# Caxson/mere-fusion

Measured on AMD Instinct MI355X. Metric: lip-sync frames/sec @256x256, higher is better.
Workload: dtype bf16x3+f16q; 1 GPU; MuseTalk step 256x256: pe(audio) + UNet(t=0) + VAE decode to uint8 frames, batch=8 latents + Whisper chunks per GPU, inputs resident in HBM (BASELINE.json configs[2]); assumed MuseTalk-v1 / sd-vae-ft-mse architecture, seeded random-init weights; batch_per_gpu=8, parallelism=1 independent replicas, sessions sharded by GPU, no collective

## Files before the change

### mere-fusion_amd/csrc/mf_attn.hip

```cpp
#include "mf_nn.h"
#include <cmath>
#include <cstdlib>

typedef __attribute__((ext_vector_type(8))) __bf16 bf16x8;
typedef __attribute__((ext_vector_type(4))) short s16x4;
typedef __attribute__((ext_vector_type(8))) short s16x8;
typedef __attribute__((ext_vector_type(4))) float f32x4;
typedef __attribute__((ext_vector_type(4))) unsigned u32x4;
typedef __attribute__((ext_vector_type(2))) unsigned u32x2;

struct AttnArgs {
    const bf16_t *q_hi, *q_lo, *k_hi, *k_lo, *v_hi, *v_lo;
    bf16_t *o_hi, *o_lo;
    int64_t q_b, k_b, v_b, o_b;
    int q_row, k_row, v_row, o_row;
    int Tq, Tk, heads, qtiles, total;
    float scale_log2e;
};

namespace {

__device__ __forceinline__ uint32_t f2bf_rne(float f) {
    return (uint32_t)__builtin_bit_cast(unsigned short, (__bf16)f);
}
__device__ __forceinline__ float bf2f_(uint32_t h16) { return __uint_as_float(h16 << 16); }

__device__ __forceinline__ s16x4 lds_tr16(const bf16_t* p) {
    return __builtin_amdgcn_ds_read_tr16_b64_v4i16((s16x4 __attribute__((address_space(3)))*)(p));
}

template <int DH, int QB, int KT, bool X3>
__global__ __launch_bounds__(256) void k_attention(const AttnArgs a) {
    constexpr int NP = X3 ? 2 : 1;
    constexpr int NK32 = (DH + 31) / 32;
    constexpr int DHP = NK32 * 32 + 8;
    constexpr int MB = (DH + 15) / 16;
    constexpr int KB = KT / 16;
    constexpr int CPR = DH / 8;
    constexpr int CH = KT * CPR;
    constexpr int RND = (CH + 255) / 256;
    static_assert(DH % 8 == 0, "head dim");
    static_assert(KT % 32 == 0, "key tile");

    __shared__ __attribute__((aligned(16))) bf16_t Ks[NP][KT][DHP];
    __shared__ __attribute__((aligned(16))) bf16_t Vs[NP][KT][DHP];

    const int tid = threadIdx.x, lane = tid & 63, l16 = lane & 15, g = lane >> 4;
    const int wave = __builtin_amdgcn_readfirstlane(tid >> 6);

    const int bid = blockIdx.x, nt = a.total;
    const int qq = nt >> 3, rr = nt & 7, xcd = bid & 7;
    const int t = (xcd < rr ? xcd * (qq + 1) : rr * (qq + 1) + (xcd - rr) * qq) + (bid >> 3);
    const int grp = t / a.qtiles, qt = t - grp * a.qtiles;
    const int b = grp / a.heads, h = grp - b * a.heads;

    const bf16_t* qp[NP] = {a.q_hi + b * a.q_b + h * DH};
    const bf16_t* kp[NP] = {a.k_hi + b * a.k_b + h * DH};
    const bf16_t* vp[NP] = {a.v_hi + b * a.v_b + h * DH};
    if constexpr (X3) {
        qp[1] = a.q_lo + b * a.q_b + h * DH;
        kp[1] = a.k_lo + b * a.k_b + h * DH;
        vp[1] = a.v_lo + b * a.v_b + h * DH;
    }

    for (int i = tid; i < NP * KT * (DHP - DH); i += 256) {
        const int r = i / (DHP - DH), c = DH + i - r * (DHP - DH);
        (&Ks[0][0][0])[r * DHP + c] = 0;
        (&Vs[0][0][0])[r * DHP + c] = 0;
    }

    const int q0 = qt * (64 * QB) + wave * (16 * QB);
    bf16x8 qf[NP][QB][NK32];
#pragma unroll
    for (int qb = 0; qb < QB; ++qb) {
        int qrow = q0 + qb * 16 + l16;
        qrow = qrow < a.Tq ? qrow : a.Tq - 1;
#pragma unroll
        for (int p = 0; p < NP; ++p) {
            const bf16_t* src = qp[p] + (int64_t)qrow * a.q_row;
#pragma unroll
            for (int ks = 0; ks < NK32; ++ks) {
// ... 28 lines not shown
#pragma unroll
        for (int r = 0; r < RND; ++r) {
            const int c = tid + r * 256;
            if (CH % 256 == 0 || c < CH) {
                const int row = c / CPR, col = c - row * CPR;
#pragma unroll
                for (int p = 0; p < NP; ++p) {
                    *reinterpret_cast<u32x4*>(&Ks[p][row][col * 8]) = pre[p][r];
                    *reinterpret_cast<u32x4*>(&Vs[p][row][col * 8]) = pre[NP + p][r];
                }
            }
        }
    };

    f32x4 oacc[MB][QB];
#pragma unroll
    for (int mb = 0; mb < MB; ++mb)
#pragma unroll
        for (int qb = 0; qb < QB; ++qb) oacc[mb][qb] = f32x4{0.f, 0.f, 0.f, 0.f};
    float m_run[QB], l_run[QB];
#pragma unroll
    for (int qb = 0; qb < QB; ++qb) { m_run[qb] = -INFINITY; l_run[qb] = 0.f; }

    const int ntiles = (a.Tk + KT - 1) / KT;
    load_tile(0);
    for (int tile = 0; tile < ntiles; ++tile) {
        __syncthreads();
        store_tile();
        __syncthreads();
        if (tile + 1 < ntiles) load_tile(tile + 1);

        f32x4 s[KB][QB];
#pragma unroll
        for (int kb = 0; kb < KB; ++kb) {
#pragma unroll
            for (int qb = 0; qb < QB; ++qb) s[kb][qb] = f32x4{0.f, 0.f, 0.f, 0.f};
            const int krow = kb * 16 + l16;
#pragma unroll
            for (int ks = 0; ks < NK32; ++ks) {
                const bf16x8 khi = *reinterpret_cast<const bf16x8*>(&Ks[0][krow][ks * 32 + g * 8]);
                bf16x8 klo;
                if constexpr (X3) klo = *reinterpret_cast<const bf16x8*>(&Ks[NP - 1][krow][ks * 32 + g * 8]);
#pragma unroll
                for (int qb = 0; qb < QB; ++qb) {
                    if constexpr (X3) {
                        s[kb][qb] = __builtin_amdgcn_mfma_f32_16x16x32_bf16(klo, qf[0][qb][ks], s[kb][qb], 0, 0, 0);
                        s[kb][qb] = __builtin_amdgcn_mfma_f32_16x16x32_bf16(khi, qf[NP - 1][qb][ks], s[kb][qb], 0, 0, 0);
                    }
                    s[kb][qb] = __builtin_amdgcn_mfma_f32_16x16x32_bf16(khi, qf[0][qb][ks], s[kb][qb], 0, 0, 0);
                }
            }
        }

        const bool last = (tile + 1) * KT > a.Tk;
#pragma unroll
        for (int qb = 0; qb < QB; ++qb) {
            float mx = -INFINITY;
#pragma unroll
            for (int kb = 0; kb < KB; ++kb)
#pragma unroll
                for (int i = 0; i < 4; ++i) {
                    float v = s[kb][qb][i] * a.scale_log2e;
                    if (last && tile * KT + kb * 16 + g * 4 + i >= a.Tk) v = -INFINITY;
                    s[kb][qb][i] = v;
                    mx = fmaxf(mx, v);
                }
            mx = fmaxf(mx, __shfl_xor(mx, 16));
            mx = fmaxf(mx, __shfl_xor(mx, 32));
            const float m_new = fmaxf(m_run[qb], mx);
            const float alpha = __builtin_amdgcn_exp2f(m_run[qb] - m_new);
            m_run[qb] = m_new;
            float ps = 0.f;
#pragma unroll
            for (int kb = 0; kb < KB; ++kb)
#pragma unroll
                for (int i = 0; i < 4; ++i) {
                    const float p = __builtin_amdgcn_exp2f(s[kb][qb][i] - m_new);
                    s[kb][qb][i] = p;
                    ps += p;
                }
            l_run[qb] = l_run[qb] * alpha + ps;
#pragma unroll
            for (int mb = 0; mb < MB; ++mb)
#pragma unroll
                for (int i = 0; i < 4; ++i) oacc[mb][qb][i] *= alpha;
        }

#pragma unroll
        for (int pi = 0; pi < KB / 2; ++pi) {
            s16x8 phi[QB], plo[QB];
#pragma unroll
            for (int qb = 0; qb < QB; ++qb)
#pragma unroll
                for (int j = 0; j < 8; ++j) {
                    const float p = s[2 * pi + (j >> 2)][qb][j & 3];
                    const uint32_t hb = f2bf_rne(p);
                    phi[qb][j] = (short)hb;
                    if constexpr (X3) plo[qb][j] = (short)f2bf_rne(p - bf2f_(hb));
                }
            const int vrow = pi * 32 + g * 4 + (l16 >> 2), vcol = (l16 & 3) * 4;
#pragma unroll
            for (int mb = 0; mb < MB; ++mb) {
                const s16x4 a0 = lds_tr16(&Vs[0][vrow][mb * 16 + vcol]);
                const s16x4 a1 = lds_tr16(&Vs[0][vrow + 16][mb * 16 + vcol]);
                const s16x8 vhi = {a0[0], a0[1], a0[2], a0[3], a1[0], a1[1], a1[2], a1[3]};
                s16x8 vlo;
                if constexpr (X3) {
                    const s16x4 b0 = lds_tr16(&Vs[NP - 1][vrow][mb * 16 + vcol]);
                    const s16x4 b1 = lds_tr16(&Vs[NP - 1][vrow + 16][mb * 16 + vcol]);
                    vlo = s16x8{b0[0], b0[1], b0[2], b0[3], b1[0], b1[1], b1[2], b1[3]};
                }
#pragma unroll
                for (int qb = 0; qb < QB; ++qb) {
                    if constexpr (X3) {
                        oacc[mb][qb] = __builtin_amdgcn_mfma_f32_16x16x32_bf16(__builtin_bit_cast(bf16x8, vlo), __builtin_bit_cast(bf16x8, phi[qb]), oacc[mb][qb], 0, 0, 0);
                        oacc[mb][qb] = __builtin_amdgcn_mfma_f32_16x16x32_bf16(__builtin_bit_cast(bf16x8, vhi), __builtin_bit_cast(bf16x8, plo[qb]), oacc[mb][qb], 0, 0, 0);
                    }
                    oacc[mb][qb] = __builtin_amdgcn_mfma_f32_16x16x32_bf16(__builtin_bit_cast(bf16x8, vhi), __builtin_bit_cast(bf16x8, phi[qb]), oacc[mb][qb], 0, 0, 0);
                }
            }
        }
    }

    bf16_t* oh = a.o_hi + b * a.o_b + h * DH;
    bf16_t* ol = X3 ? a.o_lo + b * a.o_b + h * DH : nullptr;
#pragma unroll
    for (int qb = 0; qb < QB; ++qb) {
        float l = l_run[qb];
        l += __shfl_xor(l, 16);
        l += __shfl_xor(l, 32);
        const float inv = 1.f / l;
        const int qrow = q0 + qb * 16 + l16;
        if (qrow >= a.Tq) continue;
#pragma unroll
        for (int mb = 0; mb < MB; ++mb) {
            const int d = mb * 16 + g * 4;
            if (d >= DH) continue;
            float v[4];
            uint32_t hb[4];
#pragma unroll
            for (int i = 0; i < 4; ++i) { v[i] = oacc[mb][qb][i] * inv; hb[i] = f2bf_rne(v[i]); }
            const int64_t o = (int64_t)qrow * a.o_row + d;
            *reinterpret_cast<u32x2*>(oh + o) = u32x2{hb[0] | (hb[1] << 16), hb[2] | (hb[3] << 16)};
            if constexpr (X3) {
                uint32_t lb[4];
#pragma unroll
                for (int i = 0; i < 4; ++i) lb[i] = f2bf_rne(v[i] - bf2f_(hb[i]));
                *reinterpret_cast<u32x2*>(ol + o) = u32x2{lb[0] | (lb[1] << 16), lb[2] | (lb[3] << 16)};
            }
        }
    }
}

template <int DH, int QB, int KT>
int launch_prec(const AttnArgs& a, bool x3, hipStream_t s) {
    if (x3)
        hipLaunchKernelGGL((k_attention<DH, QB, KT, true>), dim3(a.total), dim3(256), 0, s, a);
    else
        hipLaunchKernelGGL((k_attention<DH, QB, KT, false>), dim3(a.total), dim3(256), 0, s, a);
    MF_HIP(hipGetLastError());
    return MF_OK;
}

template <int DH, int KT>
int launch_qb(AttnArgs& a, int groups, bool x3, hipStream_t s) {
    const bool wide = (int64_t)groups * ((a.Tq + 127) / 128) >= 512;
    if (DH <= 80 && wide) {
        a.qtiles = (a.Tq + 127) / 128;
        a.total = groups * a.qtiles;
        return launch_prec<DH, (DH <= 80 ? 2 : 1), KT>(a, x3, s);
    }
    a.qtiles = (a.Tq + 63) / 64;
    a.total = groups * a.qtiles;
    return launch_prec<DH, 1, KT>(a, x3, s);
}

}

bool mf_attention_supported(int dh) { return dh == 40 || dh == 64 || dh == 80 || dh == 160; }

int mf_attention(const ActView& q, const ActView& k, const ActView& v, const ActView& out, int heads, int batch, int precision,
                 hipStream_t s, int tq, int tk) {
    const int C = q.C, dh = C / heads;
    MF_REQUIRE(heads > 0 && C % heads == 0 && k.C == C && v.C == C && out.C == C, "attention: channel mismatch");
    MF_REQUIRE(mf_attention_supported(dh), "attention: no fused kernel for head dim %d", dh);
    for (const ActBuf* b : {q.buf, k.buf, v.buf, out.buf})
        MF_REQUIRE(b->halo == 0 || b->H == 1, "attention: needs contiguous token buffers");
    MF_REQUIRE(q.coff % 8 == 0 && k.coff % 8 == 0 && v.coff % 8 == 0 && out.coff % 8 == 0, "attention: views must start on 8-channel groups");
    const bool x3 = precision == MF_PREC_BF16X3;
    AttnArgs a{};
    const int64_t qo = mf_interior(*q.buf) + q.coff, ko = mf_interior(*k.buf) + k.coff, vo = mf_interior(*v.buf) + v.coff,
                  oo = mf_interior(*out.buf) + out.coff;
    a.q_hi = q.buf->hi + qo; a.k_hi = k.buf->hi + ko; a.v_hi = v.buf->hi + vo; a.o_hi = out.buf->hi + oo;
    if (x3) {
        a.q_lo = q.buf->lo + qo; a.k_lo = k.buf->lo + ko; a.v_lo = v.buf->lo + vo; a.o_lo = out.buf->lo + oo;
    }
    a.q_b = q.buf->per_batch(); a.k_b = k.buf->per_batch(); a.v_b = v.buf->per_batch(); a.o_b = out.buf->per_batch();
    a.q_row = q.buf->C; a.k_row = k.buf->C; a.v_row = v.buf->C; a.o_row = out.buf->C;
    a.Tq = q.buf->H * q.buf->W; a.Tk = k.buf->H * k.buf->W; a.heads = heads;
    MF_REQUIRE(a.Tq > 0 && a.Tk > 0 && v.buf->H * v.buf->W == a.Tk && out.buf->H * out.buf->W == a.Tq, "attention: token count mismatch");
    MF_REQUIRE(tq >= 0 && tq <= a.Tq && tk >= 0 && tk <= a.Tk, "attention: prefix (%d queries, %d keys) exceeds the sequences (%d, %d)", tq, tk, a.Tq, a.Tk);
    if (tq > 0) a.Tq = tq;
    if (tk > 0) a.Tk = tk;
    a.scale_log2e = (float)(1.4426950408889634 / std::sqrt((double)dh));
    const int groups = batch * heads;
    switch (dh) {
        case 40: return launch_qb<40, 64>(a, groups, x3, s);
        case 64: return launch_qb<64, 64>(a, groups, x3, s);
        case 80: return launch_qb<80, 64>(a, groups, x3, s);
        case 160: return launch_qb<160, 32>(a, groups, x3, s);
    }
    return MF_ERR_INVALID;
}

namespace {
struct TokBuf {
    ActBuf b;
    ~TokBuf() {
        if (b.hi) (void)hipFree(b.hi);
        if (b.lo) (void)hipFree(b.lo);
    }
    int alloc(int C, int T, int batch, bool x3) {
        b.C = C; b.H = 1; b.W = T; b.halo = 0;
        const size_t bytes = ((size_t)batch * b.per_batch() + 64) * sizeof(bf16_t);
        MF_HIP(hipMalloc(&b.hi, bytes));
        MF_HIP(hipMemset(b.hi, 0, bytes));
        if (x3) {
            MF_HIP(hipMalloc(&b.lo, bytes));
            MF_HIP(hipMemset(b.lo, 0, bytes));
        }
        return MF_OK;
    }
};
}

extern "C" int mf_attention_forward(const float* q, const float* k, const float* v, float* out, int batch, int tq, int tk,
                                    int heads, int head_dim, int precision, void* stream) {
    MF_REQUIRE(q && k && v && out, "attention_forward: null argument");
    MF_REQUIRE(batch > 0 && tq > 0 && tk > 0 && heads > 0, "attention_forward: batch=%d tq=%d tk=%d heads=%d", batch, tq, tk, heads);
    MF_REQUIRE(precision == MF_PREC_BF16 || precision == MF_PREC_BF16X3, "attention_forward: unknown precision %d", precision);
    MF_REQUIRE(mf_attention_supported(head_dim), "attention_forward: head_dim %d has no fused kernel (40, 64, 80, 160)", head_dim);
    hipStream_t s = (hipStream_t)stream;
    const bool x3 = precision == MF_PREC_BF16X3;
    const int C = heads * head_dim;
    TokBuf bq, bk, bv, bo;
    int rc;
    if ((rc = bq.alloc(C, tq, batch, x3)) || (rc = bk.alloc(C, tk, batch, x3)) || (rc = bv.alloc(C, tk, batch, x3)) ||
        (rc = bo.alloc(C, tq, batch, x3)))
        return rc;
    MF_HIP(hipDeviceSynchronize());
    if ((rc = mf_rows_from_f32(q, nullptr, ActView{&bq.b, 0, C}, batch, s))) return rc;
    if ((rc = mf_rows_from_f32(k, nullptr, ActView{&bk.b, 0, C}, batch, s))) return rc;
    if ((rc = mf_rows_from_f32(v, nullptr, ActView{&bv.b, 0, C}, batch, s))) return rc;
    if ((rc = mf_attention(ActView{&bq.b, 0, C}, ActView{&bk.b, 0, C}, ActView{&bv.b, 0, C}, ActView{&bo.b, 0, C}, heads, batch, precision, s)))
        return rc;
    if ((rc = mf_rows_to_f32(ActView{&bo.b, 0, C}, out, batch, s))) return rc;
    MF_HIP(hipStreamSynchronize(s));
    return MF_OK;
}
```

### mere-fusion_amd/csrc/mf_musetalk.hip

```cpp
#include "mf_nn.h"
#include "mf_aux.h"
#include <algorithm>
#include <cmath>
#include <cstdlib>
#include <cstring>
#include <functional>
#include <map>
#include <set>
#include <memory>
#include <string>
#include <tuple>
#include <vector>

namespace {

typedef std::function<int(int, hipStream_t)> Op;

static int gn_silu_to_q(const ActView& x, const float* dg, const float* db, int groups, float eps, double* st, float* scale, float* shift, const ActBuf& tq, int B,
                        hipStream_t s, bool have_stats, const float* post, bool fuse) {
    const ActBuf& xb = *x.buf;
    if (fuse && (xb.H * xb.W) % 64 == 0) {
        if (!have_stats) { const int rc = mf_groupnorm_stats(x, groups, st, B, s); if (rc) return rc; }
        return mf_affine_silu_to_act_q(x, scale, shift, 1, tq, B, s, post, st, dg, db, groups, eps);
    }
// ... 305 lines not shown
        stats_forget(out.buf);
        push(name, epi ? "k_gn_apply (statistics from the producer's epilogue)" : "k_gn_stats+k_gn_apply", 0.0,
             [=](int B, hipStream_t s) { return mf_groupnorm(in, out, dg, db, groups, eps, silu, st, B, s, epi); });
        return MF_OK;
    }
    std::vector<std::unique_ptr<TailConv>> tails;
    int gn_conv_tail(const std::string& gname, const std::string& cname, ActView x, ActView out, int cin, int cout, int groups, float eps) {
        static const bool fuse = !(getenv("MF_TAIL_FUSE") && atoi(getenv("MF_TAIL_FUSE")) == 0);
        if (!fuse || !mf_tail_conv_supported(cin, cout, precision) || x.buf->H % 16 || x.buf->W % 16 || (x.buf->H / 16) * (x.buf->W / 16) < 32) {
            ActBuf* t = buf(cin, x.buf->H, x.buf->W, 1);
            if (!t) return MF_ERR_HIP;
            const ActView tv{t, 0, cin};
            const int rc = gn(gname, x, tv, groups, eps, true);
            return rc ? rc : conv(cname, tv, out, cin, cout, 3, 1, 1, 0, ActView{});
        }
        const float* g = T(gname + ".weight", cin);
        const float* b = T(gname + ".bias", cin);
        const float* w = T(cname + ".weight", (int64_t)cout * cin * 9);
        const float* cb = T(cname + ".bias", cout);
        if (!g || !b || !w || !cb) return MF_ERR_INVALID;
        float* dg = upload(g, cin);
        float* db = upload(b, cin);
        if (!dg || !db) return MF_ERR_HIP;
        if (gn_count >= GN_MAX_OPS) { err = "more GroupNorm layers than GN_MAX_OPS"; return MF_ERR_INVALID; }
        double* st = gn_stats + (size_t)(gn_count++) * gn_slice;
        tails.emplace_back(new TailConv());
        TailConv* tp = tails.back().get();
        const int rc = mf_tail_conv_create(tp, w, cb, cin, cout);
        if (rc) return rc;
        const bool epi = take_stats(x, groups, st);
        stats_forget(out.buf);
        push(gname + " + " + cname, epi ? "k_gn_conv3_tail (statistics from the producer's epilogue)" : "k_gn_stats+k_gn_conv3_tail",
             2.0 * 9 * cin * cout * x.buf->H * x.buf->W,
             [=](int B, hipStream_t s) { return mf_gn_conv3_tail(*tp, x, dg, db, groups, eps, true, st, epi, out, B, s); });
        return MF_OK;
    }
    int ln(const std::string& name, ActView in, ActView out) {
        const float* g = T(name + ".weight", in.C);
        const float* b = T(name + ".bias", in.C);
        if (!g || !b) return MF_ERR_INVALID;
        float* dg = upload(g, in.C);
        float* db = upload(b, in.C);
        if (!dg || !db) return MF_ERR_HIP;
        push(name, "k_layernorm", 0.0, [=](int B, hipStream_t s) { return mf_layernorm(in, out, dg, db, 1e-5f, B, s); });
        return MF_OK;
    }
    int attention(ActView q, ActView k, ActView v, ActView out, int heads) {
        const int C = q.C, dh = C / heads;
        const int Tq = q.buf->H * q.buf->W, Tk = k.buf->H * k.buf->W;
        if (q.buf->halo || k.buf->halo || v.buf->halo || out.buf->halo || dh % 8 || k.C != C || v.C != C || out.C != C) {
            err = "attention: needs contiguous token buffers and a head dim that is a multiple of 8";
            return MF_ERR_INVALID;
        }
        if (mf_attention_supported(dh)) {
            const int prec = precision;
            push("attention " + std::to_string(Tq) + "x" + std::to_string(Tk) + " heads " + std::to_string(heads) + " dh " + std::to_string(dh),
                 "k_attention", 4.0 * Tq * Tk * C, [=](int B, hipStream_t s) { return mf_attention(q, k, v, out, heads, B, prec, s); });
            return MF_OK;
        }
        const int Tk8 = (Tk + 7) / 8 * 8, Tk64 = (Tk + 63) / 64 * 64;
        auto key = std::make_tuple(dh, Tq, Tk, heads);
        if (!attn_plans.count(key)) {
            ConvPlan* ps = new_plan();
            ConvPlan* pv = new_plan();
            int rc;
            if ((rc = mf_gemm_plan_create_grouped(ps, dh, Tk, Tq, cap * heads, precision))) return rc;
            if ((rc = mf_gemm_plan_create_grouped(pv, Tk64, dh, Tq, cap * heads, precision))) return rc;
            for (ConvPlan* p : {ps, pv}) {
                std::vector<int> goff(p->goff_total);
                for (int g = 0; g < p->goff_total; ++g) goff[g] = (g < p->cin_pad / 8 ? g : 0) * 8;
                MF_HIP(hipMemcpy(p->goff, goff.data(), goff.size() * sizeof(int), hipMemcpyHostToDevice));
                p->bound_in_ld = 1; p->bound_in_wp = 1;
            }
            attn_plans[key] = {ps, pv};
        }
        ConvPlan* ps = attn_plans[key].first;
        ConvPlan* pv = attn_plans[key].second;
        ActBuf* sc = tmp("attn.scores", Tk8, heads, Tq, 0);
        ActBuf* pm = tmp("attn.probs", Tk64, heads, Tq, 0);
        if (!sc || !pm) return MF_ERR_HIP;
        const float scale = 1.0f / std::sqrt((float)dh);
        const bool x3 = precision == MF_PREC_BF16X3;
        push("attention " + std::to_string(Tq) + "x" + std::to_string(Tk) + " heads " + std::to_string(heads) + " dh " + std::to_string(dh),
             "pack+gemm+softmax+pack+gemm", 4.0 * Tq * Tk * C, [=](int B, hipStream_t s) {
            int rc;
            if ((rc = mf_pack_b_grouped(ps, k.buf->hi + k.coff, x3 ? k.buf->lo + k.coff : nullptr, k.buf->per_batch(), dh,
                                        k.buf->C, 1, Tk, dh, B * heads, heads, s))) return rc;
            GroupedGemm g{};
            g.x_hi = q.buf->hi + q.coff; g.x_lo = x3 ? q.buf->lo + q.coff : nullptr;
            g.zx_b = q.buf->per_batch(); g.zx_h = dh; g.x_row = q.buf->C;
            g.y_hi = sc->hi; g.y_lo = sc->lo; g.zy_b = sc->per_batch(); g.zy_h = (int64_t)Tq * sc->C; g.y_row = sc->C;
            g.M = Tq; g.groups = B * heads; g.heads = heads;
            if ((rc = mf_gemm_grouped_launch(ps, g, s))) return rc;
            if ((rc = mf_softmax_rows(ActView{sc, 0, Tk}, ActView{pm, 0, pm->C}, Tk, scale, B, s))) return rc;
            if ((rc = mf_pack_b_grouped(pv, v.buf->hi + v.coff, x3 ? v.buf->lo + v.coff : nullptr, v.buf->per_batch(), dh,
                                        1, v.buf->C, dh, Tk, B * heads, heads, s))) return rc;
            GroupedGemm o{};
            o.x_hi = pm->hi; o.x_lo = pm->lo; o.zx_b = pm->per_batch(); o.zx_h = (int64_t)Tq * pm->C; o.x_row = pm->C;
            o.y_hi = out.buf->hi + out.coff; o.y_lo = x3 ? out.buf->lo + out.coff : nullptr;
            o.zy_b = out.buf->per_batch(); o.zy_h = dh; o.y_row = out.buf->C;
            o.M = Tq; o.groups = B * heads; o.heads = heads;
            return mf_gemm_grouped_launch(pv, o, s);
        });
        return MF_OK;
    }

    int resnet(const std::string& p, ActView x, ActView y, int cin, int cout, int groups, float eps, const std::vector<float>* temb_act) {
        const int H = x.buf->H, W = x.buf->W;
        ActBuf *t1 = tmp("rn.t1", cin, H, W, 1), *c1 = tmp("rn.c1", cout, H, W, 1), *t2 = tmp("rn.t2", cout, H, W, 1);
        if (!t1 || !c1 || !t2) return MF_ERR_HIP;
        int rc;
        std::vector<float> tb;
        if (temb_act && has(p + ".time_emb_proj.weight")) {
            const int td = (int)temb_act->size();
            const float* w = T(p + ".time_emb_proj.weight", (int64_t)cout * td);
            const float* b = T(p + ".time_emb_proj.bias", cout);
            if (!w || !b) return MF_ERR_INVALID;
            tb.resize(cout);
            for (int o = 0; o < cout; ++o) {
                double a = b[o];
                for (int i = 0; i < td; ++i) a += (double)w[(size_t)o * td + i] * (*temb_act)[i];
                tb[o] = (float)a;
            }
        }
        ActView res = x;
        int sc_op = -1;
        if (has(p + ".conv_shortcut.weight")) {
            ActBuf* sc = tmp("rn.sc", cout, H, W, 1);
            if (!sc) return MF_ERR_HIP;
            if ((rc = conv(p + ".conv_shortcut", x, ActView{sc, 0, cout}, cin, cout, 1, 1, 0, 0, ActView{}))) return rc;
            res = ActView{sc, 0, cout};
            sc_op = (int)ops.size() - 1;
            mark_side(sc_op);
        } else if (cin != cout) {
            err = p + ": cin != cout but no conv_shortcut in the state dict";
            return MF_ERR_INVALID;
        }
        if ((rc = gn_conv(p + ".norm1", p + ".conv1", x, t1, ActView{c1, 0, cout}, cin, cout, groups, eps, ActView{}, tb.empty() ? nullptr : &tb))) return rc;
        if (sc_op >= 0) join_here(sc_op);
        return gn_conv(p + ".norm2", p + ".conv2", ActView{c1, 0, cout}, t2, y, cout, cout, groups, eps, res);
    }

    int transformer(const std::string& p, ActView x, ActView y, int C, int heads, int groups, ActView ctx) {
        const int H = x.buf->H, W = x.buf->W, X = ctx.C;
        ActBuf *g0 = tmp("xf.gn", C, H, W, 0), *hA = tmp("xf.hA", C, H, W, 0), *hB = tmp("xf.hB", C, H, W, 0);
        ActBuf *nb = tmp("xf.ln", C, H, W, 0), *qkv = tmp("xf.qkv", 3 * C, H, W, 0), *ao = tmp("xf.ao", C, H, W, 0);
        ActBuf *kv = tmp("xf.kv", 2 * C, ctx.buf->H, ctx.buf->W, 0), *gg = tmp("xf.geglu", 4 * C, H, W, 0);
        if (!g0 || !hA || !hB || !nb || !qkv || !ao || !kv || !gg) return MF_ERR_HIP;
        const std::string t = p + ".transformer_blocks.0";
        int rc;
        if ((rc = gn(p + ".norm", x, ActView{g0, 0, C}, groups, 1e-6f, false))) return rc;
        if ((rc = conv(p + ".proj_in", ActView{g0, 0, C}, ActView{hA, 0, C}, C, C, 1, 1, 0, 0, ActView{}))) return rc;
        double *st1 = ln_slot(hA), *st2 = ln_slot(hB), *st3 = ln_slot(hA);
        const bool fold = st1 && st2 && st3;
        if (fold) { last_plan->ln_out = st1; if ((rc = ln_fold_next(t + ".norm1", C, st1))) return rc; }
        else if ((rc = ln(t + ".norm1", ActView{hA, 0, C}, ActView{nb, 0, C}))) return rc;
// ... 682 lines not shown
```

### mere-fusion_amd/csrc/mf_nn.h

```cpp
#pragma once
#include "mf_conv.h"

int mf_layernorm(const ActView& x, const ActView& y, const float* gamma, const float* beta, float eps, int batch,
                 hipStream_t s, int tokens = 0, int act = 0);

int mf_softmax_rows(const ActView& scores, const ActView& probs, int n_keys, float scale, int batch, hipStream_t s);

int mf_pack_b(ConvPlan* plan, const bf16_t* src_hi, const bf16_t* src_lo, int64_t stride_n, int64_t stride_k, int N,
              int K, hipStream_t s);

int mf_gemm_plan_create(ConvPlan* p, int K, int N, int T, int precision);

int mf_rows_to_f32(const ActView& x, float* dst, int batch, hipStream_t s);
int mf_rows_to_f32_layered(const ActView& x, float* dst, int batch, int tokens, int layer, int n_layers, hipStream_t s);

int mf_rows_from_f32(const float* src, const float* addend, const ActView& y, int batch, hipStream_t s);

int mf_zero_f64(double* p, int n, hipStream_t s);
int mf_groupnorm_affine(const ActView& x, const float* gamma, const float* beta, int groups, float eps, double* stats, float* scale, float* shift,
                        int batch, hipStream_t s, bool have_stats = false);
int mf_groupnorm(const ActView& x, const ActView& y, const float* gamma, const float* beta, int groups, float eps,
                 bool silu, double* stats, int batch, hipStream_t s, bool have_stats = false);

struct TailConv { int cin = 0, cout = 0; bf16_t* w = nullptr; float* bias = nullptr; };
bool mf_tail_conv_supported(int cin, int cout, int precision);
int mf_tail_conv_create(TailConv* p, const float* weight, const float* bias, int cin, int cout);
void mf_tail_conv_destroy(TailConv* p);
int mf_gn_conv3_tail(const TailConv& p, const ActView& x, const float* gamma, const float* beta, int groups, float eps, bool silu, double* stats,
                     bool have_stats, const ActView& out, int batch, hipStream_t s);

int mf_geglu(const ActView& x, const ActView& y, int batch, hipStream_t s);

int mf_pack_b_grouped(ConvPlan* plan, const bf16_t* src_hi, const bf16_t* src_lo, int64_t sb, int64_t sh, int64_t stride_n,
                      int64_t stride_k, int N, int K, int groups, int heads, hipStream_t s);
int mf_gemm_plan_create_grouped(ConvPlan* p, int K, int N, int T, int groups, int precision);

int mf_vae_post_u8(const ActView& x, uint8_t* dst, int batch, hipStream_t s);

bool mf_attention_supported(int dh);
int mf_attention(const ActView& q, const ActView& k, const ActView& v, const ActView& out, int heads, int batch, int precision,
                 hipStream_t s, int tq = 0, int tk = 0);

inline int64_t mf_interior(const ActBuf& b) { return ((int64_t)b.halo * b.Wp() + b.halo) * b.C; }
```

Measured before the change: 454.6 frames/s.

## Add split-head-dim fused attention kernel for head dim 512 in VAE

Adds k_attention_wide, a fused flash-style attention kernel for head dim 512 (the VAE mid-block attention). It splits the head dimension across four waves and reduces the partial QK scores through shared memory, replacing the previous pack+GEMM+softmax+pack+GEMM composite path. The online softmax is also refactored with compile-time options: folding the scale into an FMA, packed bf16 conversion, and skipping the output rescale when the running max is unchanged. The cost is extra block-wide syncs and LDS traffic per key tile, and a single 256-thread block per query tile may limit overlap.

```diff
diff --git a/mere-fusion_amd/csrc/mf_attn.hip b/mere-fusion_amd/csrc/mf_attn.hip
--- a/mere-fusion_amd/csrc/mf_attn.hip
+++ b/mere-fusion_amd/csrc/mf_attn.hip
@@ -1,6 +1,11 @@
 #include "mf_nn.h"
 #include <cmath>
 #include <cstdlib>
+#include <vector>
+
+#ifndef MF_ATTN_LOOP
+#define MF_ATTN_LOOP 7
+#endif
 
 typedef __attribute__((ext_vector_type(8))) __bf16 bf16x8;
 typedef __attribute__((ext_vector_type(4))) short s16x4;
@@ -8,6 +13,8 @@
 typedef __attribute__((ext_vector_type(4))) float f32x4;
 typedef __attribute__((ext_vector_type(4))) unsigned u32x4;
 typedef __attribute__((ext_vector_type(2))) unsigned u32x2;
+typedef __attribute__((ext_vector_type(2))) float f32x2;
+typedef __attribute__((ext_vector_type(2))) __bf16 bf16x2;
 
 struct AttnArgs {
     const bf16_t *q_hi, *q_lo, *k_hi, *k_lo, *v_hi, *v_lo;
@@ -27,6 +34,112 @@
 
 __device__ __forceinline__ s16x4 lds_tr16(const bf16_t* p) {
     return __builtin_amdgcn_ds_read_tr16_b64_v4i16((s16x4 __attribute__((address_space(3)))*)(p));
+}
+__device__ __forceinline__ uint32_t pk_bf16(float a, float b) {
+    return __builtin_bit_cast(uint32_t, __builtin_convertvector(f32x2{a, b}, bf16x2));
+}
+
+template <int KB, int QB, int MB>
+__device__ __forceinline__ void online_softmax(f32x4 (&s)[KB][QB], f32x4 (&oacc)[MB][QB], float (&m_run)[QB], float (&l_run)[QB], float c, bool last,
+                                               int key0, int Tk, int g) {
+    constexpr bool fold = MF_ATTN_LOOP & 1, skip = MF_ATTN_LOOP & 4;
+#pragma unroll
+    for (int qb = 0; qb < QB; ++qb) {
+        float mx = -INFINITY;
+#pragma unroll
+        for (int kb = 0; kb < KB; ++kb)
+#pragma unroll
+            for (int i = 0; i < 4; ++i) {
+                float v = fold ? s[kb][qb][i] : s[kb][qb][i] * c;
+                if (last && key0 + kb * 16 + g * 4 + i >= Tk) v = -INFINITY;
+                s[kb][qb][i] = v;
+                mx = fmaxf(mx, v);
+            }
+        mx = fmaxf(mx, __shfl_xor(mx, 16));
+        mx = fmaxf(mx, __shfl_xor(mx, 32));
+        const float m_new = fmaxf(m_run[qb], mx);
+        const float mc = fold ? m_new * c : m_new;
+        const float alpha = __builtin_amdgcn_exp2f((fold ? m_run[qb] * c : m_run[qb]) - mc);
+        const bool raised = __any(m_new != m_run[qb]);
+        m_run[qb] = m_new;
+        float ps = 0.f;
+#pragma unroll
+        for (int kb = 0; kb < KB; ++kb)
+#pragma unroll
+            for (int i = 0; i < 4; ++i) {
+                const float p = __builtin_amdgcn_exp2f(fold ? fmaf(s[kb][qb][i], c, -mc) : s[kb][qb][i] - mc);
+                s[kb][qb][i] = p;
+                ps += p;
+            }
+        l_run[qb] = l_run[qb] * alpha + ps;
+        if (!skip || raised) {
+#pragma unroll
+            for (int mb = 0; mb < MB; ++mb)
+#pragma unroll
+                for (int i = 0; i < 4; ++i) oacc[mb][qb][i] *= alpha;
+        }
+    }
+}
+
+template <int KB, int QB, bool X3>
+__device__ __forceinline__ void split_p(const f32x4 (&s)[KB][QB], int pi, bf16x8 (&phi)[QB], bf16x8 (&plo)[QB]) {
+#pragma unroll
+    for (int qb = 0; qb < QB; ++qb) {
+        if constexpr ((MF_ATTN_LOOP & 2) != 0) {
+            u32x4 h, l;
+#pragma unroll
+            for (int jp = 0; jp < 4; ++jp) {
+                const float p0 = s[2 * pi + (jp >> 1)][qb][(jp & 1) * 2], p1 = s[2 * pi + (jp >> 1)][qb][(jp & 1) * 2 + 1];
+                const uint32_t w = pk_bf16(p0, p1);
+                h[jp] = w;
+                if constexpr (X3) l[jp] = pk_bf16(p0 - __uint_as_float(w << 16), p1 - __uint_as_float(w & 0xffff0000u));
+            }
+            phi[qb] = __builtin_bit_cast(bf16x8, h);
+            if constexpr (X3) plo[qb] = __builtin_bit_cast(bf16x8, l);
+        } else {
+            s16x8 h, l;
+#pragma unroll
+            for (int j = 0; j < 8; ++j) {
+                const float p = s[2 * pi + (j >> 2)][qb][j & 3];
+                const uint32_t hb = f2bf_rne(p);
+                h[j] = (short)hb;
+                if constexpr (X3) l[j] = (short)f2bf_rne(p - bf2f_(hb));
+            }
+            phi[qb] = __builtin_bit_cast(bf16x8, h);
+            if constexpr (X3) plo[qb] = __builtin_bit_cast(bf16x8, l);
+        }
+    }
+}
+
+template <int MB, int QB, int DH, bool X3>
+__device__ __forceinline__ void store_o(const f32x4 (&oacc)[MB][QB], const float (&l_run)[QB], bf16_t* oh, bf16_t* ol, int q0, int Tq, int o_row, int l16,
+                                        int g) {
+#pragma unroll
+    for (int qb = 0; qb < QB; ++qb) {
+        float l = l_run[qb];
+        l += __shfl_xor(l, 16);
+        l += __shfl_xor(l, 32);
+        const float inv = 1.f / l;
+        const int qrow = q0 + qb * 16 + l16;
+        if (qrow >= Tq) continue;
+#pragma unroll
+        for (int mb = 0; mb < MB; ++mb) {
+            const int d = mb * 16 + g * 4;
+            if (d >= DH) continue;
+            float v[4];
+            uint32_t hb[4];
+#pragma unroll
+            for (int i = 0; i < 4; ++i) { v[i] = oacc[mb][qb][i] * inv; hb[i] = f2bf_rne(v[i]); }
+            const int64_t o = (int64_t)qrow * o_row + d;
+            *reinterpret_cast<u32x2*>(oh + o) = u32x2{hb[0] | (hb[1] << 16), hb[2] | (hb[3] << 16)};
+            if constexpr (X3) {
+                uint32_t lb[4];
+#pragma unroll
+                for (int i = 0; i < 4; ++i) lb[i] = f2bf_rne(v[i] - bf2f_(hb[i]));
+                *reinterpret_cast<u32x2*>(ol + o) = u32x2{lb[0] | (lb[1] << 16), lb[2] | (lb[3] << 16)};
+            }
+        }
+    }
 }
 
 template <int DH, int QB, int KT, bool X3>
@@ -161,52 +274,12 @@
             }
         }
 
-        const bool last = (tile + 1) * KT > a.Tk;
-#pragma unroll
-        for (int qb = 0; qb < QB; ++qb) {
-            float mx = -INFINITY;
-#pragma unroll
-            for (int kb = 0; kb < KB; ++kb)
-#pragma unroll
-                for (int i = 0; i < 4; ++i) {
-                    float v = s[kb][qb][i] * a.scale_log2e;
-                    if (last && tile * KT + kb * 16 + g * 4 + i >= a.Tk) v = -INFINITY;
-                    s[kb][qb][i] = v;
-                    mx = fmaxf(mx, v);
-                }
-            mx = fmaxf(mx, __shfl_xor(mx, 16));
-            mx = fmaxf(mx, __shfl_xor(mx, 32));
-            const float m_new = fmaxf(m_run[qb], mx);
-            const float alpha = __builtin_amdgcn_exp2f(m_run[qb] - m_new);
-            m_run[qb] = m_new;
-            float ps = 0.f;
-#pragma unroll
-            for (int kb = 0; kb < KB; ++kb)
-#pragma unroll
-                for (int i = 0; i < 4; ++i) {
-                    const float p = __builtin_amdgcn_exp2f(s[kb][qb][i] - m_new);
-                    s[kb][qb][i] = p;
-                    ps += p;
-                }
-            l_run[qb] = l_run[qb] * alpha + ps;
-#pragma unroll
-            for (int mb = 0; mb < MB; ++mb)
-#pragma unroll
-                for (int i = 0; i < 4; ++i) oacc[mb][qb][i] *= alpha;
-        }
+        online_softmax<KB, QB, MB>(s, oacc, m_run, l_run, a.scale_log2e, (tile + 1) * KT > a.Tk, tile * KT, a.Tk, g);
 
 #pragma unroll
         for (int pi = 0; pi < KB / 2; ++pi) {
-            s16x8 phi[QB], plo[QB];
-#pragma unroll
-            for (int qb = 0; qb < QB; ++qb)
-#pragma unroll
-                for (int j = 0; j < 8; ++j) {
-                    const float p = s[2 * pi + (j >> 2)][qb][j & 3];
-                    const uint32_t hb = f2bf_rne(p);
-                    phi[qb][j] = (short)hb;
-                    if constexpr (X3) plo[qb][j] = (short)f2bf_rne(p - bf2f_(hb));
-                }
+            bf16x8 phi[QB], plo[QB];
+            split_p<KB, QB, X3>(s, pi, phi, plo);
             const int vrow = pi * 32 + g * 4 + (l16 >> 2), vcol = (l16 & 3) * 4;
 #pragma unroll
             for (int mb = 0; mb < MB; ++mb) {
@@ -222,43 +295,179 @@
 #pragma unroll
                 for (int qb = 0; qb < QB; ++qb) {
                     if constexpr (X3) {
-                        oacc[mb][qb] = __builtin_amdgcn_mfma_f32_16x16x32_bf16(__builtin_bit_cast(bf16x8, vlo), __builtin_bit_cast(bf16x8, phi[qb]), oacc[mb][qb], 0, 0, 0);
-                        oacc[mb][qb] = __builtin_amdgcn_mfma_f32_16x16x32_bf16(__builtin_bit_cast(bf16x8, vhi), __builtin_bit_cast(bf16x8, plo[qb]), oacc[mb][qb], 0, 0, 0);
+                        oacc[mb][qb] = __builtin_amdgcn_mfma_f32_16x16x32_bf16(__builtin_bit_cast(bf16x8, vlo), phi[qb], oacc[mb][qb], 0, 0, 0);
+                        oacc[mb][qb] = __builtin_amdgcn_mfma_f32_16x16x32_bf16(__builtin_bit_cast(bf16x8, vhi), plo[qb], oacc[mb][qb], 0, 0, 0);
                     }
-                    oacc[mb][qb] = __builtin_amdgcn_mfma_f32_16x16x32_bf16(__builtin_bit_cast(bf16x8, vhi), __builtin_bit_cast(bf16x8, phi[qb]), oacc[mb][qb], 0, 0, 0);
-                }
-            }
-        }
-    }
-
-    bf16_t* oh = a.o_hi + b * a.o_b + h * DH;
-    bf16_t* ol = X3 ? a.o_lo + b * a.o_b + h * DH : nullptr;
+                    oacc[mb][qb] = __builtin_amdgcn_mfma_f32_16x16x32_bf16(__builtin_bit_cast(bf16x8, vhi), phi[qb], oacc[mb][qb], 0, 0, 0);
+                }
+            }
+        }
+    }
+
+    store_o<MB, QB, DH, X3>(oacc, l_run, a.o_hi + b * a.o_b + h * DH, X3 ? a.o_lo + b * a.o_b + h * DH : nullptr, q0, a.Tq, a.o_row, l16, g);
+}
+
+template <int DH, bool X3>
+__global__ __launch_bounds__(256) void k_attention_wide(const AttnArgs a) {
+    constexpr int NP = X3 ? 2 : 1;
+    constexpr int QB = 2, KT = 32, KB = KT / 16;
+    constexpr int DW = DH / 4;
+    constexpr int NKS = DW / 32;
+    constexpr int MB = DW / 16;
+    constexpr int DWP = DW + 8;
+    constexpr int CPR = DW / 8;
+    constexpr int RND = KT * CPR / 64;
+    static_assert(DW % 32 == 0 && (KT * CPR) % 64 == 0, "head dim");
+
+    __shared__ __attribute__((aligned(16))) bf16_t Vs[4][NP][KT][DWP];
+    __shared__ __attribute__((aligned(16))) f32x4 Sp[4][KB][QB][64];
+
+    const int tid = threadIdx.x, lane = tid & 63, l16 = lane & 15, g = lane >> 4;
+    const int wave = __builtin_amdgcn_readfirstlane(tid >> 6);
+
+    const int bid = blockIdx.x, nt = a.total;
+    const int qq = nt >> 3, rr = nt & 7, xcd = bid & 7;
+    const int t = (xcd < rr ? xcd * (qq + 1) : rr * (qq + 1) + (xcd - rr) * qq) + (bid >> 3);
+    const int grp = t / a.qtiles, qt = t - grp * a.qtiles;
+    const int b = grp / a.heads, h = grp - b * a.heads;
+    const int c0 = h * DH + wave * DW;
+
+    const bf16_t* qp[NP] = {a.q_hi + b * a.q_b + c0};
+    const bf16_t* kp[NP] = {a.k_hi + b * a.k_b + c0};
+    const bf16_t* vp[NP] = {a.v_hi + b * a.v_b + c0};
+    if constexpr (X3) {
+        qp[1] = a.q_lo + b * a.q_b + c0;
+        kp[1] = a.k_lo + b * a.k_b + c0;
+        vp[1] = a.v_lo + b * a.v_b + c0;
+    }
+    const u32x4 z = {0u, 0u, 0u, 0u};
+
+    const int q0 = qt * (16 * QB);
+    bf16x8 qf[NP][QB][NKS];
 #pragma unroll
     for (int qb = 0; qb < QB; ++qb) {
-        float l = l_run[qb];
-        l += __shfl_xor(l, 16);
-        l += __shfl_xor(l, 32);
-        const float inv = 1.f / l;
-        const int qrow = q0 + qb * 16 + l16;
-        if (qrow >= a.Tq) continue;
+        int qrow = q0 + qb * 16 + l16;
+        qrow = qrow < a.Tq ? qrow : a.Tq - 1;
+#pragma unroll
+        for (int p = 0; p < NP; ++p)
+#pragma unroll
+            for (int ks = 0; ks < NKS; ++ks) {
+                u32x4 raw = *reinterpret_cast<const u32x4*>(qp[p] + (int64_t)qrow * a.q_row + ks * 32 + g * 8);
+                asm volatile("" : "+v"(raw));
+                qf[p][qb][ks] = __builtin_bit_cast(bf16x8, raw);
+            }
+    }
+
+    u32x4 kpre[NP][KB][NKS], vpre[NP][RND];
+    auto load_tile = [&](int tile) __attribute__((always_inline)) {
+#pragma unroll
+        for (int kb = 0; kb < KB; ++kb) {
+            const int key = tile * KT + kb * 16 + l16;
+            const bool ok = key < a.Tk;
+#pragma unroll
+            for (int p = 0; p < NP; ++p)
+#pragma unroll
+                for (int ks = 0; ks < NKS; ++ks)
+                    kpre[p][kb][ks] = ok ? *reinterpret_cast<const u32x4*>(kp[p] + (int64_t)key * a.k_row + ks * 32 + g * 8) : z;
+        }
+#pragma unroll
+        for (int r = 0; r < RND; ++r) {
+            const int c = lane + r * 64, row = c / CPR, col = c - row * CPR;
+            const int key = tile * KT + row;
+            const bool ok = key < a.Tk;
+#pragma unroll
+            for (int p = 0; p < NP; ++p) vpre[p][r] = ok ? *reinterpret_cast<const u32x4*>(vp[p] + (int64_t)key * a.v_row + col * 8) : z;
+        }
+    };
+
+    f32x4 oacc[MB][QB];
+#pragma unroll
+    for (int mb = 0; mb < MB; ++mb)
+#pragma unroll
+        for (int qb = 0; qb < QB; ++qb) oacc[mb][qb] = f32x4{0.f, 0.f, 0.f, 0.f};
+    float m_run[QB], l_run[QB];
+#pragma unroll
+    for (int qb = 0; qb < QB; ++qb) { m_run[qb] = -INFINITY; l_run[qb] = 0.f; }
+
+    const int ntiles = (a.Tk + KT - 1) / KT;
+    load_tile(0);
+    for (int tile = 0; tile < ntiles; ++tile) {
+        __syncthreads();
+#pragma unroll
+        for (int r = 0; r < RND; ++r) {
+            const int c = lane + r * 64, row = c / CPR, col = c - row * CPR;
+#pragma unroll
+            for (int p = 0; p < NP; ++p) *reinterpret_cast<u32x4*>(&Vs[wave][p][row][col * 8]) = vpre[p][r];
+        }
+        bf16x8 kf[NP][KB][NKS];
+#pragma unroll
+        for (int p = 0; p < NP; ++p)
+#pragma unroll
+            for (int kb = 0; kb < KB; ++kb)
+#pragma unroll
+                for (int ks = 0; ks < NKS; ++ks) kf[p][kb][ks] = __builtin_bit_cast(bf16x8, kpre[p][kb][ks]);
+        if (tile + 1 < ntiles) load_tile(tile + 1);
+
+#pragma unroll
+        for (int kb = 0; kb < KB; ++kb)
+#pragma unroll
+            for (int qb = 0; qb < QB; ++qb) {
+                f32x4 sp = {0.f, 0.f, 0.f, 0.f};
+#pragma unroll
+                for (int ks = 0; ks < NKS; ++ks) {
+                    if constexpr (X3) {
+                        sp = __builtin_amdgcn_mfma_f32_16x16x32_bf16(kf[NP - 1][kb][ks], qf[0][qb][ks], sp, 0, 0, 0);
+                        sp = __builtin_amdgcn_mfma_f32_16x16x32_bf16(kf[0][kb][ks], qf[NP - 1][qb][ks], sp, 0, 0, 0);
+                    }
+                    sp = __builtin_amdgcn_mfma_f32_16x16x32_bf16(kf[0][kb][ks], qf[0][qb][ks], sp, 0, 0, 0);
+                }
+                Sp[wave][kb][qb][lane] = sp;
+            }
+        __syncthreads();
+
+        f32x4 s[KB][QB];
+#pragma unroll
+        for (int kb = 0; kb < KB; ++kb)
+#pragma unroll
+            for (int qb = 0; qb < QB; ++qb) {
+                f32x4 v = Sp[0][kb][qb][lane];
+#pragma unroll
+                for (int w = 1; w < 4; ++w) {
+                    const f32x4 u = Sp[w][kb][qb][lane];
+#pragma unroll
+                    for (int i = 0; i < 4; ++i) v[i] = v[i] + mf_opaque(u[i]);
+                }
+                s[kb][qb] = v;
+            }
+
+        online_softmax<KB, QB, MB>(s, oacc, m_run, l_run, a.scale_log2e, (tile + 1) * KT > a.Tk, tile * KT, a.Tk, g);
+
+        bf16x8 phi[QB], plo[QB];
+        split_p<KB, QB, X3>(s, 0, phi, plo);
+        const int vrow = g * 4 + (l16 >> 2), vcol = (l16 & 3) * 4;
 #pragma unroll
         for (int mb = 0; mb < MB; ++mb) {
-            const int d = mb * 16 + g * 4;
-            if (d >= DH) continue;
-            float v[4];
-            uint32_t hb[4];
-#pragma unroll
-            for (int i = 0; i < 4; ++i) { v[i] = oacc[mb][qb][i] * inv; hb[i] = f2bf_rne(v[i]); }
-            const int64_t o = (int64_t)qrow * a.o_row + d;
-            *reinterpret_cast<u32x2*>(oh + o) = u32x2{hb[0] | (hb[1] << 16), hb[2] | (hb[3] << 16)};
+            const s16x4 a0 = lds_tr16(&Vs[wave][0][vrow][mb * 16 + vcol]);
+            const s16x4 a1 = lds_tr16(&Vs[wave][0][vrow + 16][mb * 16 + vcol]);
+            const bf16x8 vhi = __builtin_bit_cast(bf16x8, s16x8{a0[0], a0[1], a0[2], a0[3], a1[0], a1[1], a1[2], a1[3]});
+            bf16x8 vlo;
             if constexpr (X3) {
-                uint32_t lb[4];
-#pragma unroll
-                for (int i = 0; i < 4; ++i) lb[i] = f2bf_rne(v[i] - bf2f_(hb[i]));
-                *reinterpret_cast<u32x2*>(ol + o) = u32x2{lb[0] | (lb[1] << 16), lb[2] | (lb[3] << 16)};
-            }
-        }
-    }
+                const s16x4 b0 = lds_tr16(&Vs[wave][NP - 1][vrow][mb * 16 + vcol]);
+                const s16x4 b1 = lds_tr16(&Vs[wave][NP - 1][vrow + 16][mb * 16 + vcol]);
+                vlo = __builtin_bit_cast(bf16x8, s16x8{b0[0], b0[1], b0[2], b0[3], b1[0], b1[1], b1[2], b1[3]});
+            }
+#pragma unroll
+            for (int qb = 0; qb < QB; ++qb) {
+                if constexpr (X3) {
+                    oacc[mb][qb] = __builtin_amdgcn_mfma_f32_16x16x32_bf16(vlo, phi[qb], oacc[mb][qb], 0, 0, 0);
+                    oacc[mb][qb] = __builtin_amdgcn_mfma_f32_16x16x32_bf16(vhi, plo[qb], oacc[mb][qb], 0, 0, 0);
+                }
+                oacc[mb][qb] = __builtin_amdgcn_mfma_f32_16x16x32_bf16(vhi, phi[qb], oacc[mb][qb], 0, 0, 0);
+            }
+        }
+    }
+
+    store_o<MB, QB, DW, X3>(oacc, l_run, a.o_hi + b * a.o_b + c0, X3 ? a.o_lo + b * a.o_b + c0 : nullptr, q0, a.Tq, a.o_row, l16, g);
 }
 
 template <int DH, int QB, int KT>
@@ -284,9 +493,26 @@
     return launch_prec<DH, 1, KT>(a, x3, s);
 }
 
-}
-
-bool mf_attention_supported(int dh) { return dh == 40 || dh == 64 || dh == 80 || dh == 160; }
+template <int DH>
+int launch_wide(AttnArgs& a, int groups, bool x3, hipStream_t s) {
+    a.qtiles = (a.Tq + 31) / 32;
+    a.total = groups * a.qtiles;
+    if (x3)
+        hipLaunchKernelGGL((k_attention_wide<DH, true>), dim3(a.total), dim3(256), 0, s, a);
+    else
+        hipLaunchKernelGGL((k_attention_wide<DH, false>), dim3(a.total), dim3(256), 0, s, a);
+    MF_HIP(hipGetLastError());
+    return MF_OK;
+}
+
+}
+
+bool mf_attention_supported(int dh, bool wide) { return dh == 40 || dh == 64 || dh == 80 || dh == 160 || (wide && dh == 512); }
+
+bool mf_attention_wide_enabled() {
+    const char* e = getenv("MF_ATTN_WIDE");
+    return !e || atoi(e) != 0;
+}
 
 int mf_attention(const ActView& q, const ActView& k, const ActView& v, const ActView& out, int heads, int batch, int precision,
                  hipStream_t s, int tq, int tk) {
@@ -318,8 +544,47 @@
         case 64: return launch_qb<64, 64>(a, groups, x3, s);
         case 80: return launch_qb<80, 64>(a, groups, x3, s);
         case 160: return launch_qb<160, 32>(a, groups, x3, s);
+        case 512: return launch_wide<512>(a, groups, x3, s);
     }
     return MF_ERR_INVALID;
+}
+
+int mf_attention_composite_plans(ConvPlan* ps, ConvPlan* pv, int dh, int Tq, int Tk, int groups, int precision) {
+    int rc;
+    if ((rc = mf_gemm_plan_create_grouped(ps, dh, Tk, Tq, groups, precision))) return rc;
+    if ((rc = mf_gemm_plan_create_grouped(pv, (Tk + 63) / 64 * 64, dh, Tq, groups, precision))) return rc;
+    for (ConvPlan* p : {ps, pv}) {
+        std::vector<int> goff(p->goff_total);
+        for (int g = 0; g < p->goff_total; ++g) goff[g] = (g < p->cin_pad / 8 ? g : 0) * 8;
+        MF_HIP(hipMemcpy(p->goff, goff.data(), goff.size() * sizeof(int), hipMemcpyHostToDevice));
+        p->bound_in_ld = 1; p->bound_in_wp = 1;
+    }
+    return MF_OK;
+}
+
+int mf_attention_composite(ConvPlan* ps, ConvPlan* pv, const ActBuf* sc, const ActBuf* pm, const ActView& q, const ActView& k, const ActView& v,
+                           const ActView& out, int heads, int batch, int precision, hipStream_t s) {
+    const int dh = q.C / heads, Tq = q.buf->H * q.buf->W, Tk = k.buf->H * k.buf->W;
+    const float scale = 1.0f / std::sqrt((float)dh);
+    const bool x3 = precision == MF_PREC_BF16X3;
+    int rc;
+    if ((rc = mf_pack_b_grouped(ps, k.buf->hi + k.coff, x3 ? k.buf->lo + k.coff : nullptr, k.buf->per_batch(), dh,
+                                k.buf->C, 1, Tk, dh, batch * heads, heads, s))) return rc;
+    GroupedGemm g{};
+    g.x_hi = q.buf->hi + q.coff; g.x_lo = x3 ? q.buf->lo + q.coff : nullptr;
+    g.zx_b = q.buf->per_batch(); g.zx_h = dh; g.x_row = q.buf->C;
+    g.y_hi = sc->hi; g.y_lo = sc->lo; g.zy_b = sc->per_batch(); g.zy_h = (int64_t)Tq * sc->C; g.y_row = sc->C;
+    g.M = Tq; g.groups = batch * heads; g.heads = heads;
+    if ((rc = mf_gemm_grouped_launch(ps, g, s))) return rc;
+    if ((rc = mf_softmax_rows(ActView{const_cast<ActBuf*>(sc), 0, Tk}, ActView{const_cast<ActBuf*>(pm), 0, pm->C}, Tk, scale, batch, s))) return rc;
+    if ((rc = mf_pack_b_grouped(pv, v.buf->hi + v.coff, x3 ? v.buf->lo + v.coff : nullptr, v.buf->per_batch(), dh,
+                                1, v.buf->C, dh, Tk, batch * heads, heads, s))) return rc;
+    GroupedGemm o{};
+    o.x_hi = pm->hi; o.x_lo = pm->lo; o.zx_b = pm->per_batch(); o.zx_h = (int64_t)Tq * pm->C; o.x_row = pm->C;
+    o.y_hi = out.buf->hi + out.coff; o.y_lo = x3 ? out.buf->lo + out.coff : nullptr;
+    o.zy_b = out.buf->per_batch(); o.zy_h = dh; o.y_row = out.buf->C;
+    o.M = Tq; o.groups = batch * heads; o.heads = heads;
+    return mf_gemm_grouped_launch(pv, o, s);
 }
 
 namespace {
@@ -329,8 +594,8 @@
         if (b.hi) (void)hipFree(b.hi);
         if (b.lo) (void)hipFree(b.lo);
     }
-    int alloc(int C, int T, int batch, bool x3) {
-        b.C = C; b.H = 1; b.W = T; b.halo = 0;
+    int alloc(int C, int T, int batch, bool x3, int H = 1) {
+        b.C = C; b.H = H; b.W = T; b.halo = 0;
         const size_t bytes = ((size_t)batch * b.per_batch() + 64) * sizeof(bf16_t);
         MF_HIP(hipMalloc(&b.hi, bytes));
         MF_HIP(hipMemset(b.hi, 0, bytes));
@@ -348,7 +613,7 @@
     MF_REQUIRE(q && k && v && out, "attention_forward: null argument");
     MF_REQUIRE(batch > 0 && tq > 0 && tk > 0 && heads > 0, "attention_forward: batch=%d tq=%d tk=%d heads=%d", batch, tq, tk, heads);
     MF_REQUIRE(precision == MF_PREC_BF16 || precision == MF_PREC_BF16X3, "attention_forward: unknown precision %d", precision);
-    MF_REQUIRE(mf_attention_supported(head_dim), "attention_forward: head_dim %d has no fused kernel (40, 64, 80, 160)", head_dim);
+    MF_REQUIRE(mf_attention_supported(head_dim), "attention_forward: head_dim %d has no fused kernel (40, 64, 80, 160, 512)", head_dim);
     hipStream_t s = (hipStream_t)stream;
     const bool x3 = precision == MF_PREC_BF16X3;
     const int C = heads * head_dim;
@@ -361,8 +626,26 @@
     if ((rc = mf_rows_from_f32(q, nullptr, ActView{&bq.b, 0, C}, batch, s))) return rc;
     if ((rc = mf_rows_from_f32(k, nullptr, ActView{&bk.b, 0, C}, batch, s))) return rc;
     if ((rc = mf_rows_from_f32(v, nullptr, ActView{&bv.b, 0, C}, batch, s))) return rc;
-    if ((rc = mf_attention(ActView{&bq.b, 0, C}, ActView{&bk.b, 0, C}, ActView{&bv.b, 0, C}, ActView{&bo.b, 0, C}, heads, batch, precision, s)))
+    if (mf_attention_supported(head_dim, mf_attention_wide_enabled())) {
+        if ((rc = mf_attention(ActView{&bq.b, 0, C}, ActView{&bk.b, 0, C}, ActView{&bv.b, 0, C}, ActView{&bo.b, 0, C}, heads, batch, precision, s)))
+            return rc;
+    } else {
+        ConvPlan ps, pv;
+        TokBuf sc, pm;
+        if ((rc = mf_attention_composite_plans(&ps, &pv, head_dim, tq, tk, batch * heads, precision)) || (rc = sc.alloc((tk + 7) / 8 * 8, tq, batch, x3, heads)) ||
+            (rc = pm.alloc((tk + 63) / 64 * 64, tq, batch, x3, heads)) ||
+            (rc = mf_attention_composite(&ps, &pv, &sc.b, &pm.b, ActView{&bq.b, 0, C}, ActView{&bk.b, 0, C}, ActView{&bv.b, 0, C}, ActView{&bo.b, 0, C},
+                                         heads, batch, precision, s))) {
+            mf_conv_plan_destroy(&ps);
+            mf_conv_plan_destroy(&pv);
+            return rc;
+        }
+        rc = mf_rows_to_f32(ActView{&bo.b, 0, C}, out, batch, s);
+        MF_HIP(hipStreamSynchronize(s));
+        mf_conv_plan_destroy(&ps);
+        mf_conv_plan_destroy(&pv);
         return rc;
+    }
     if ((rc = mf_rows_to_f32(ActView{&bo.b, 0, C}, out, batch, s))) return rc;
     MF_HIP(hipStreamSynchronize(s));
     return MF_OK;
diff --git a/mere-fusion_amd/csrc/mf_musetalk.hip b/mere-fusion_amd/csrc/mf_musetalk.hip
--- a/mere-fusion_amd/csrc/mf_musetalk.hip
+++ b/mere-fusion_amd/csrc/mf_musetalk.hip
@@ -381,56 +381,30 @@
             err = "attention: needs contiguous token buffers and a head dim that is a multiple of 8";
             return MF_ERR_INVALID;
         }
-        if (mf_attention_supported(dh)) {
+        const bool wide = mf_attention_wide_enabled();
+        const std::string name = "attention " + std::to_string(Tq) + "x" + std::to_string(Tk) + " heads " + std::to_string(heads) + " dh " + std::to_string(dh);
+        if (mf_attention_supported(dh, wide)) {
             const int prec = precision;
-            push("attention " + std::to_string(Tq) + "x" + std::to_string(Tk) + " heads " + std::to_string(heads) + " dh " + std::to_string(dh),
-                 "k_attention", 4.0 * Tq * Tk * C, [=](int B, hipStream_t s) { return mf_attention(q, k, v, out, heads, B, prec, s); });
+            push(name, dh > 160 ? "k_attention_wide" : "k_attention", 4.0 * Tq * Tk * C,
+                 [=](int B, hipStream_t s) { return mf_attention(q, k, v, out, heads, B, prec, s); });
             return MF_OK;
         }
-        const int Tk8 = (Tk + 7) / 8 * 8, Tk64 = (Tk + 63) / 64 * 64;
         auto key = std::make_tuple(dh, Tq, Tk, heads);
         if (!attn_plans.count(key)) {
             ConvPlan* ps = new_plan();
             ConvPlan* pv = new_plan();
-            int rc;
-            if ((rc = mf_gemm_plan_create_grouped(ps, dh, Tk, Tq, cap * heads, precision))) return rc;
-            if ((rc = mf_gemm_plan_create_grouped(pv, Tk64, dh, Tq, cap * heads, precision))) return rc;
-            for (ConvPlan* p : {ps, pv}) {
-                std::vector<int> goff(p->goff_total);
-                for (int g = 0; g < p->goff_total; ++g) goff[g] = (g < p->cin_pad / 8 ? g : 0) * 8;
-                MF_HIP(hipMemcpy(p->goff, goff.data(), goff.size() * sizeof(int), hipMemcpyHostToDevice));
-                p->bound_in_ld = 1; p->bound_in_wp = 1;
-            }
+            const int rc = mf_attention_composite_plans(ps, pv, dh, Tq, Tk, cap * heads, precision);
+            if (rc) return rc;
             attn_plans[key] = {ps, pv};
         }
         ConvPlan* ps = attn_plans[key].first;
         ConvPlan* pv = attn_plans[key].second;
-        ActBuf* sc = tmp("attn.scores", Tk8, heads, Tq, 0);
-        ActBuf* pm = tmp("attn.probs", Tk64, heads, Tq, 0);
+        ActBuf* sc = tmp("attn.scores", (Tk + 7) / 8 * 8, heads, Tq, 0);
+        ActBuf* pm = tmp("attn.probs", (Tk + 63) / 64 * 64, heads, Tq, 0);
         if (!sc || !pm) return MF_ERR_HIP;
-        const float scale = 1.0f / std::sqrt((float)dh);
-        const bool x3 = precision == MF_PREC_BF16X3;
-        push("attention " + std::to_string(Tq) + "x" + std::to_string(Tk) + " heads " + std::to_string(heads) + " dh " + std::to_string(dh),
-             "pack+gemm+softmax+pack+gemm", 4.0 * Tq * Tk * C, [=](int B, hipStream_t s) {
-            int rc;
-            if ((rc = mf_pack_b_grouped(ps, k.buf->hi + k.coff, x3 ? k.buf->lo + k.coff : nullptr, k.buf->per_batch(), dh,
-                                        k.buf->C, 1, Tk, dh, B * heads, heads, s))) return rc;
-            GroupedGemm g{};
-            g.x_hi = q.buf->hi + q.coff; g.x_lo = x3 ? q.buf->lo + q.coff : nullptr;
-            g.zx_b = q.buf->per_batch(); g.zx_h = dh; g.x_row = q.buf->C;
-            g.y_hi = sc->hi; g.y_lo = sc->lo; g.zy_b = sc->per_batch(); g.zy_h = (int64_t)Tq * sc->C; g.y_row = sc->C;
-            g.M = Tq; g.groups = B * heads; g.heads = heads;
-            if ((rc = mf_gemm_grouped_launch(ps, g, s))) return rc;
-            if ((rc = mf_softmax_rows(ActView{sc, 0, Tk}, ActView{pm, 0, pm->C}, Tk, scale, B, s))) return rc;
-            if ((rc = mf_pack_b_grouped(pv, v.buf->hi + v.coff, x3 ? v.buf->lo + v.coff : nullptr, v.buf->per_batch(), dh,
-                                        1, v.buf->C, dh, Tk, B * heads, heads, s))) return rc;
-            GroupedGemm o{};
-            o.x_hi = pm->hi; o.x_lo = pm->lo; o.zx_b = pm->per_batch(); o.zx_h = (int64_t)Tq * pm->C; o.x_row = pm->C;
-            o.y_hi = out.buf->hi + out.coff; o.y_lo = x3 ? out.buf->lo + out.coff : nullptr;
-            o.zy_b = out.buf->per_batch(); o.zy_h = dh; o.y_row = out.buf->C;
-            o.M = Tq; o.groups = B * heads; o.heads = heads;
-            return mf_gemm_grouped_launch(pv, o, s);
-        });
+        const int prec = precision;
+        push(name, "pack+gemm+softmax+pack+gemm", 4.0 * Tq * Tk * C,
+             [=](int B, hipStream_t s) { return mf_attention_composite(ps, pv, sc, pm, q, k, v, out, heads, B, prec, s); });
         return MF_OK;
     }
 
diff --git a/mere-fusion_amd/csrc/mf_nn.h b/mere-fusion_amd/csrc/mf_nn.h
--- a/mere-fusion_amd/csrc/mf_nn.h
+++ b/mere-fusion_amd/csrc/mf_nn.h
@@ -37,8 +37,13 @@
 
 int mf_vae_post_u8(const ActView& x, uint8_t* dst, int batch, hipStream_t s);
 
-bool mf_attention_supported(int dh);
+bool mf_attention_supported(int dh, bool wide = true);
+bool mf_attention_wide_enabled();
 int mf_attention(const ActView& q, const ActView& k, const ActView& v, const ActView& out, int heads, int batch, int precision,
                  hipStream_t s, int tq = 0, int tk = 0);
 
+int mf_attention_composite_plans(ConvPlan* ps, ConvPlan* pv, int dh, int Tq, int Tk, int groups, int precision);
+int mf_attention_composite(ConvPlan* ps, ConvPlan* pv, const ActBuf* sc, const ActBuf* pm, const ActView& q, const ActView& k, const ActView& v,
+                           const ActView& out, int heads, int batch, int precision, hipStream_t s);
+
 inline int64_t mf_interior(const ActBuf& b) { return ((int64_t)b.halo * b.Wp() + b.halo) * b.C; }
```

New measurement: 451.1 frames/s. About the same (-0.8%).
